# Sue1347/SMSUT-MedicalImgSegmentation

Hardware: AMD Instinct MI355X
Metric: slices/sec uganConsisTrainer step @256x256 (higher is better)
Workload: dtype f32

## Files before the change

### smsut-medicalimgsegmentation_amd/csrc/conv_mfma.hip

```cpp
#include "common.h"
#include "conv_wino.h"
#include "conv_wgrad_rr.h"
#include <stdlib.h>
#include <type_traits>

namespace {

typedef float f32x4 __attribute__((ext_vector_type(4)));

constexpr int TPB = 256;
constexpr int TW = 16;
constexpr int CK = 16;
constexpr int SPIX = 24;

#ifdef SMSUT_STAMPS
__device__ unsigned long long* g_stamps = nullptr;
__device__ int g_stamp_base = 0;
#define STAMP(i)                                                                                       \
  if (g_stamps && lane == 0 && stamp_wg >= g_stamp_base && stamp_wg < g_stamp_base + 512)                \
    g_stamps[(((stamp_wg - g_stamp_base) * 4 + wave) * 16) + (i)] = __builtin_amdgcn_s_memtime();
#else
#define STAMP(i)
#endif

// ... 151 lines not shown
        else *(float4*)(w_s + w_dst[i]) = rw[i];
      }
    }
    __syncthreads();
    if (step < 2) { STAMP(3 + 4 * step); }
    if (step + 1 < nsteps) prefetch(step + 1);
    if (step < 2) { STAMP(4 + 4 * step); }
    if constexpr (CKW == 32) {
#pragma unroll
      for (int tap = 0; tap < KK; ++tap) {
        const int kh = tap / KS, kw = tap % KS;
        h8 a[MR], b[NR];
#pragma unroll
        for (int i = 0; i < MR; ++i)
          a[i] = *(const h8*)(in_h + (((wm * MR + i) * RPT + a_row + kh) * IW + a_col + kw) * PXH + 8 * kq);
#pragma unroll
        for (int j = 0; j < NR; ++j)
          b[j] = *(const h8*)(w_h + ((size_t)tap * CO_T + (wn * NR + j) * 16 + lm) * WRH + 8 * kq);
#pragma unroll
        for (int i = 0; i < MR; ++i)
#pragma unroll
          for (int j = 0; j < NR; ++j) acc[i][j] = mfma32h(a[i], b[j], acc[i][j]);
      }
    } else if constexpr (F16 && SMSUT_F16_X32) {
      const bool hi = kq >= 2;
      const int ko = 8 * (kq & 1);
      const h8 zero8 = {(_Float16)0.f, (_Float16)0.f, (_Float16)0.f, (_Float16)0.f, (_Float16)0.f, (_Float16)0.f, (_Float16)0.f, (_Float16)0.f};
#pragma unroll
      for (int p = 0; p < (KK + 1) / 2; ++p) {
        const bool solo = 2 * p + 1 >= KK;
        const int tlo = 2 * p, thi = solo ? 2 * p : 2 * p + 1;
        const int tap = hi ? thi : tlo;
        const int kh = hi ? thi / KS : tlo / KS, kw = hi ? thi % KS : tlo % KS;
        h8 a[MR], b[NR];
#pragma unroll
        for (int i = 0; i < MR; ++i) {
          a[i] = *(const h8*)(in_h + (((wm * MR + i) * RPT + a_row + kh) * IW + a_col + kw) * SPIXH + ko);
          if (solo && hi) a[i] = zero8;
        }
#pragma unroll
        for (int j = 0; j < NR; ++j) {
          b[j] = *(const h8*)(w_h + ((size_t)tap * CO_T + (wn * NR + j) * 16 + lm) * WROWH + ko);
          if (solo && hi) b[j] = zero8;
        }
#pragma unroll
        for (int i = 0; i < MR; ++i)
#pragma unroll
          for (int j = 0; j < NR; ++j) acc[i][j] = mfma32h(a[i], b[j], acc[i][j]);
      }
    } else if constexpr (F16) {
#pragma unroll
      for (int tap = 0; tap < KK; ++tap) {
        const int kh = tap / KS, kw = tap % KS;
        h4 a[MR], b[NR];
#pragma unroll
        for (int i = 0; i < MR; ++i)
          a[i] = *(const h4*)(in_h + (((wm * MR + i) * RPT + a_row + kh) * IW + a_col + kw) * SPIXH + 4 * kq);
#pragma unroll
        for (int j = 0; j < NR; ++j)
          b[j] = *(const h4*)(w_h + ((size_t)tap * CO_T + (wn * NR + j) * 16 + lm) * WROWH + 4 * kq);
#pragma unroll
        for (int i = 0; i < MR; ++i)
#pragma unroll
          for (int j = 0; j < NR; ++j) acc[i][j] = mfma16h(a[i], b[j], acc[i][j]);
      }
    } else
#pragma unroll
    for (int tap = 0; tap < KK; ++tap) {
      const int kh = tap / KS, kw = tap % KS;
      f32x4 a[MR], b[NR];
#pragma unroll
      for (int i = 0; i < MR; ++i)
        a[i] = *(const f32x4*)(in_s + (((wm * MR + i) * RPT + a_row + kh) * IW + a_col + kw) * SPIX + 4 * kq);
#pragma unroll
      for (int j = 0; j < NR; ++j)
        b[j] = *(const f32x4*)(w_s + (((tap * 4 + kq) * CO_T) + (wn * NR + j) * 16 + lm) * 4);
#pragma unroll
      for (int s = 0; s < 4; ++s)
#pragma unroll
        for (int i = 0; i < MR; ++i)
#pragma unroll
          for (int j = 0; j < NR; ++j) acc[i][j] = mfma16(a[i][s], b[j][s], acc[i][j]);
    }
    if (step < 2) { STAMP(5 + 4 * step); }
  }
  if (F16) {
#pragma unroll
    for (int i = 0; i < MR; ++i)
#pragma unroll
      for (int j = 0; j < NR; ++j) acc[i][j] *= gi;
  }
  if (stats) {
    __syncthreads();
    float* red = smem;
#pragma unroll
    for (int j = 0; j < NR; ++j) {
      float s1 = 0.f, s2 = 0.f;
#pragma unroll
      for (int i = 0; i < MR; ++i) {
#pragma unroll
        for (int r = 0; r < 4; ++r) {
          const int p = 4 * kq + r;
          const bool ok = y0 + (wm * MR + i) * RPT + p / MW < H && x0 + p % MW < W;
          const float v = ok ? acc[i][j][r] : 0.f;
          s1 += v; s2 += v * v;
        }
      }
      s1 += __shfl_xor(s1, 16, 64); s2 += __shfl_xor(s2, 16, 64);
      s1 += __shfl_xor(s1, 32, 64); s2 += __shfl_xor(s2, 32, 64);
      if (kq == 0) {
        red[(wm * CO_T + (wn * NR + j) * 16 + lm) * 2] = s1;
        red[(wm * CO_T + (wn * NR + j) * 16 + lm) * 2 + 1] = s2;
      }
    }
    __syncthreads();
    if (tid < CO_T && co0 + tid < Ndim) {
      float s1 = 0.f, s2 = 0.f;
#pragma unroll
      for (int m = 0; m < WM; ++m) { s1 += red[(m * CO_T + tid) * 2]; s2 += red[(m * CO_T + tid) * 2 + 1]; }
      float* o = stats + (((size_t)n_img * gridDim.x + tile) * Ndim + co0 + tid) * 2;
      o[0] = s1; o[1] = s2;
    }
  }
  STAMP(10);
  const int Wo = W * osc;
#pragma unroll
  for (int i = 0; i < MR; ++i) {
#pragma unroll
    for (int j = 0; j < NR; ++j) {
      const int co = co0 + (wn * NR + j) * 16 + lm;
      if (co >= Ndim) continue;
      const bool hi = y2 && co0 + (wn * NR + j) * 16 >= split;
      const int os = !y2 ? Ndim : (hi ? Ndim - split : split);
      float* yout = (hi ? y2 : y) + (size_t)n_img * H * osc * Wo * os + (hi ? co - split : co);
#pragma unroll
      for (int r = 0; r < 4; ++r) {
        const int p = 4 * kq + r;
        const int gy_ = y0 + (wm * MR + i) * RPT + p / MW, gx_ = x0 + p % MW;
        if (gy_ < H && gx_ < W) {
          float* o = yout + ((size_t)(gy_ * osc + (tapo >> 1)) * Wo + gx_ * osc + (tapo & 1)) * os;
          *o = accum ? acc[i][j][r] + *o : acc[i][j][r];
        }
      }
    }
  }
  STAMP(11);
}

__device__ __forceinline__ float aff1(float v, float m, float r, float g, float b, float slope) {
  return lrelu_f(in_affine(v, m, r, g, b), slope);
}

constexpr int SPIXW = 20;

template <int KS, int TH, int NTN, int NCH, bool STATS, bool ACC, bool BST = false, bool DUAL = false, bool INAFF = false,
          bool F16 = false, bool K8 = false, bool SC = false, bool SC2 = false, bool N8 = false, bool WINO = false, bool O16 = false, bool I16 = false,
          bool FIN = false>
__global__ void __launch_bounds__(TPB) __attribute__((amdgpu_waves_per_eu(WINO ? 2 : 1, WINO ? 2 : 8)))
conv_mfma_fwd_p(const float* __restrict__ x, const float* __restrict__ w, float* __restrict__ y, int N, int H, int W,
                int Ndim, int tiles_x, int tiles_img, int items_per_wg, int transposed, float* __restrict__ stats,
                BstRef bst = BstRef{}, float* __restrict__ y2 = nullptr, int split = 0,
                const float* __restrict__ x2 = nullptr, AffRef aff = AffRef{}, const float* __restrict__ gsc = nullptr,
                ScRef sc = ScRef{}, FinRef fin = FinRef{}) {
  static_assert(!FIN || ((STATS || BST) && !F16 && !N8), "in-launch finalize: fp32 statistics / BST forms");
  static_assert(!SC || (STATS && !ACC && !BST && !INAFF && KS == 3), "fused shortcut: forward statistics forms");
  static_assert(!(SC && F16 && (K8 || WINO)), "fused shortcut with fp16 operands: the direct 16-channel-chunk form");
  static_assert(!SC2 || (DUAL && !STATS && !ACC && !BST && !INAFF && !K8 && !SC && KS == 3), "fused shortcut data-gradient");
  static_assert(!(SC2 && F16 && (WINO || N8)), "fused shortcut data-gradient with fp16 operands: the direct form, >= 16 result channels");
  static_assert(!N8 || (NTN == 1 && !STATS && !BST && !INAFF && !F16 && !K8 && !SC), "8 result channels: plain / accumulate / SC2 data-gradient forms");
  [[maybe_unused]] const bool nok = !N8 || (threadIdx.x & 15) < 8;
  static_assert(!K8 || (NCH == 1 && !DUAL && !INAFF && !F16 && !BST), "8-channel reduction: plain / statistics / accumulate / fused-shortcut forms");
  static_assert(!WINO || (KS == 3 && TH == 16 && !F16 && !K8 && !N8), "Winograd form: 3x3, 16-row items, fp32");
  static_assert(!O16 || ((F16 || (K8 && SC)) && !ACC && (!INAFF || I16) && (STATS != BST)),
                "fp16 storage: forward statistics forms / BST data-gradient, fp16 operands (or the 8-channel fused-shortcut form)");
  static_assert(!I16 || (F16 && STATS && !BST && !DUAL && !SC), "fp16 input: plain / input-side-IN forward statistics form, fp16 operands");
  constexpr int SPX = WINO ? SPIXW : SPIX;
  constexpr int NPOS = WINO ? 16 : KS * KS;
  static_assert(!(BST && (STATS || ACC)), "BST excludes the forward statistics and the accumulate form");
  static_assert(!INAFF || (STATS && !ACC && !BST && !DUAL), "input-side IN: forward statistics form only");
  static_assert(!DUAL || NCH % 2 == 0, "virtual cat input: two equal halves of whole 16-channel chunks");
  constexpr int KST = K8 ? 8 : (DUAL ? 8 * NCH : 16 * NCH);
  constexpr int KK = KS * KS;
  constexpr int PAD = (KS - 1) / 2;
  constexpr int IH = TH + KS - 1, IW = TW + KS - 1;
  constexpr int CO_T = 16 * NTN;
  constexpr int MR = TH / 4, NR = NTN;
  constexpr int Kdim = K8 ? 8 : 16 * NCH, K4 = Kdim / 4;
  constexpr int UQ = K8 ? 2 : 4;
  constexpr int UNITS = IH * IW * UQ;
  constexpr int NI = (UNITS + TPB - 1) / TPB;
  extern __shared__ float smem[];
  float* in_s = smem;
  float* red = smem + (IH * IW + 1) * SPX;
  float* w_s = red + 2 * 4 * CO_T * 2 + 8;
  [[maybe_unused]] float* wsc_s = w_s + NPOS * Kdim * CO_T;
  [[maybe_unused]] float* red_sc = wsc_s + Kdim * CO_T;
  [[maybe_unused]] _Float16* in_h = reinterpret_cast<_Float16*>(smem);
  [[maybe_unused]] _Float16* w_h = reinterpret_cast<_Float16*>(w_s);
  [[maybe_unused]] _Float16* wsc_h = reinterpret_cast<_Float16*>(wsc_s);
  [[maybe_unused]] const float gs = (F16 && gsc) ? gsc[0] : 1.f, gi = (F16 && gsc) ? gsc[1] : 1.f;

  const int tid = threadIdx.x;
  const int lane = tid & 63, wave = tid >> 6;
  const int lm = lane & 15, kq = lane >> 4;
  const int co0 = blockIdx.y * CO_T;
  float* const yo = (y2 && co0 >= split) ? y2 : y;
  const int os = !y2 ? Ndim : (co0 >= split ? Ndim - split : split);
  const int oc0 = (y2 && co0 >= split) ? co0 - split : co0;
  const int total_items = N * tiles_img;
  const int wg = (gridDim.x & 7) == 0 ? (int)((blockIdx.x & 7) * (gridDim.x >> 3) + (blockIdx.x >> 3)) : (int)blockIdx.x;
  const int item0 = wg * items_per_wg;
  const int item1 = min(item0 + items_per_wg, total_items);
  if (item0 >= item1) return;
  const int tiles_y = tiles_img / tiles_x;
  [[maybe_unused]] const int stamp_wg = blockIdx.y == 0 ? (int)blockIdx.x : -1;
  STAMP(0);

  if constexpr (WINO) {
    for (int u = tid; u < Kdim * CO_T; u += TPB) {
      const int n = u % CO_T, ci = u / CO_T;
      const int ng = co0 + n;
      if constexpr (SC2) {
        constexpr int Kh = Kdim / 2;
        if (ci >= Kh) {
          w_s[(((size_t)(ci >> 2)) * CO_T + n) * 4 + (ci & 3)] = sc.w[(size_t)ng * Kh + (ci - Kh)];
          continue;
        }
      }
      constexpr int KROW = SC2 ? Kdim / 2 : Kdim;
      float g[3][3];
#pragma unroll
      for (int tap = 0; tap < 9; ++tap)
        g[tap / 3][tap % 3] = !(transposed || SC2) ? w[((size_t)tap * Kdim + ci) * Ndim + ng]
                                                   : w[((size_t)(8 - tap) * Ndim + ng) * KROW + ci];
      float t[4][3];
#pragma unroll
      for (int b = 0; b < 3; ++b) {
        t[0][b] = g[0][b];
        t[1][b] = 0.5f * (g[0][b] + g[1][b] + g[2][b]);
        t[2][b] = 0.5f * (g[0][b] - g[1][b] + g[2][b]);
        t[3][b] = g[2][b];
      }
#pragma unroll
      for (int a = 0; a < 4; ++a) {
        const float uu[4] = {t[a][0], 0.5f * (t[a][0] + t[a][1] + t[a][2]), 0.5f * (t[a][0] - t[a][1] + t[a][2]), t[a][2]};
#pragma unroll
        for (int b = 0; b < 4; ++b) w_s[(((size_t)(a * 4 + b) * K4 + (ci >> 2)) * CO_T + n) * 4 + (ci & 3)] = uu[b];
      }
    }
  }
  for (int u = tid; u < (WINO ? 0 : KK * K4 * CO_T); u += TPB) {
    const int n = u % CO_T;
    const int k4 = (u / CO_T) % K4;
    const int tap = u / (CO_T * K4);
    const int ng = co0 + n;
    float4 v;
    if (N8 && n >= 8) {
      v = make_float4(0.f, 0.f, 0.f, 0.f);
    } else if constexpr (SC2) {
      constexpr int Kh = Kdim / 2;
      if (k4 < K4 / 2) v = *(const float4*)(w + ((size_t)(KK - 1 - tap) * Ndim + ng) * Kh + 4 * k4);
      else if (tap == KK / 2) v = *(const float4*)(sc.w + (size_t)ng * Kh + 4 * (k4 - K4 / 2));
      else v = make_float4(0.f, 0.f, 0.f, 0.f);
    } else if (!transposed) {
      const float* p = w + ((size_t)tap * Kdim + 4 * k4) * Ndim + ng;
      v.x = p[0]; v.y = p[Ndim]; v.z = p[2 * (size_t)Ndim]; v.w = p[3 * (size_t)Ndim];
    } else {
      v = *(const float4*)(w + ((size_t)(KK - 1 - tap) * Ndim + ng) * Kdim + 4 * k4);
    }
    if (F16) *(h4*)(w_h + ((size_t)(tap * NCH + (k4 >> 2)) * CO_T + n) * WROWH + 4 * (k4 & 3)) = to_h4(v);
    else *(float4*)(w_s + (size_t)u * 4) = v;
  }
  if constexpr (SC) {
    for (int u = tid; u < K4 * CO_T; u += TPB) {
      const int n = u % CO_T, k4 = u / CO_T;
      const float* p = sc.w + (size_t)(4 * k4) * Ndim + co0 + n;
      const float4 v = make_float4(p[0], p[Ndim], p[2 * (size_t)Ndim], p[3 * (size_t)Ndim]);
      if (F16) *(h4*)(wsc_h + ((size_t)(k4 >> 2) * CO_T + n) * WROWH + 4 * (k4 & 3)) = to_h4(v);
      else *(float4*)(wsc_s + (size_t)u * 4) = v;
    }
  }

  int u_off[NI], u_lds[NI], u_flag[NI];
  float4 rin[I16 ? 1 : NI];
  [[maybe_unused]] h4 rinh[I16 ? NI : 1];
#pragma unroll
  for (int i = 0; i < NI; ++i) {
    const int u = tid + i * TPB;
    const bool real = u < UNITS;
    const int uu = real ? u : 0;
    const int q = uu % UQ, pix = uu / UQ;
    const int iy = pix / IW, ix = pix % IW;
    u_off[i] = (iy * W + ix) * KST + 4 * q;
    u_lds[i] = real ? pix * (F16 ? SPIXH : SPX) + 4 * q : IH * IW * (F16 ? SPIXH : SPX);
    u_flag[i] = (iy < PAD ? 1 : 0) | (iy >= TH + PAD ? 2 : 0) | (ix < PAD ? 4 : 0) | (ix >= TW + PAD ? 8 : 0);
  }
  const int safe_off = (PAD * W + PAD) * KST;

  int pn = item0 / tiles_img, pty, ptx;
  { const int t = item0 - pn * tiles_img; pty = t / tiles_x; ptx = t - pty * tiles_x; }
  int cn = pn, cty = pty, ctx = ptx;
  int en = pn, ety = pty, etx = ptx;
  int pflags = 0;
  bool zero[NI];
  [[maybe_unused]] float4 a_m, a_r, a_g, a_b;

  auto prefetch = [&](int c) __attribute__((always_inline)) {
    if (c == 0) pflags = (pty == 0 ? 1 : 0) | (pty == tiles_y - 1 ? 2 : 0) | (ptx == 0 ? 4 : 0) | (ptx == tiles_x - 1 ? 8 : 0);
    const int cl = DUAL ? c % (NCH / 2 > 0 ? NCH / 2 : 1) : c;
    const int base = (((pn * H + pty * TH - PAD) * W) + ptx * TW - PAD) * KST + cl * 16;
    const float* xb = ((DUAL && c >= NCH / 2) ? x2 : x) + base;
    if constexpr (I16) {
      const _Float16* xh = reinterpret_cast<const _Float16*>(x) + base;
#pragma unroll
      for (int i = 0; i < NI; ++i) {
        zero[i] = (u_flag[i] & pflags) != 0;
        rinh[i] = *(const h4*)(xh + (zero[i] ? safe_off : u_off[i]));
      }
    } else {
#pragma unroll
      for (int i = 0; i < NI; ++i) {
        zero[i] = (u_flag[i] & pflags) != 0;
        rin[i] = *(const float4*)(xb + (zero[i] ? safe_off : u_off[i]));
      }
    }
    if (INAFF) {
      const int ch = c * 16 + 4 * (tid & 3);
      a_m = *(const float4*)(aff.mean + (size_t)pn * Kdim + ch);
// ... 50 lines not shown
      for (int j = 0; j < NR; ++j) qacc[q_][j] = (f32x4){0.f, 0.f, 0.f, 0.f};
  }
  if constexpr (SC) {
#pragma unroll
    for (int i = 0; i < MR; ++i)
#pragma unroll
      for (int j = 0; j < NR; ++j) { acs[i][j] = (f32x4){0.f, 0.f, 0.f, 0.f}; pacs[i][j] = acs[i][j]; }
  }
  [[maybe_unused]] f32x4 pold[MR][NR];
  [[maybe_unused]] float nm[NR], nr[NR], ng[NR], nb[NR];
#pragma unroll
  for (int i = 0; i < MR; ++i)
#pragma unroll
    for (int j = 0; j < NR; ++j) { acc[i][j] = (f32x4){0.f, 0.f, 0.f, 0.f}; pacc[i][j] = acc[i][j]; }

  if (BST) {
#pragma unroll
    for (int j = 0; j < NR; ++j) { ng[j] = bst.gamma[co0 + j * 16 + lm]; nb[j] = bst.beta[co0 + j * 16 + lm]; }
  }
  const int o_lane = WINO ? ((wave * MR + 2 * (kq >> 1)) * W + 8 * (kq & 1)) * os + lm : ((wave * MR) * W + 4 * kq) * os + lm;
  const int red_slot = (wave * CO_T + lm) * 2;
  auto pxo = [&](int i, int r) __attribute__((always_inline)) { return WINO ? (i >> 1) * W + 2 * r + (i & 1) : i * W + r; };

  auto epilogue = [&](int par) __attribute__((always_inline)) {
    if (F16) {
#pragma unroll
      for (int i = 0; i < MR; ++i)
#pragma unroll
        for (int j = 0; j < NR; ++j) pacc[i][j] *= gi;
    }
    if (STATS || BST) {
#pragma unroll
      for (int j = 0; j < NR; ++j) {
        float s1 = 0.f, s2 = 0.f;
#pragma unroll
        for (int i = 0; i < MR; ++i)
#pragma unroll
          for (int r = 0; r < 4; ++r) {
            if (BST) {
              const float yv = pold[i][j][r];
              const float gz = pacc[i][j][r] * lrelu_mask(in_affine(yv, nm[j], nr[j], ng[j], nb[j]), bst.slope);
              pacc[i][j][r] = gz;
              s1 += gz; s2 += gz * ((yv - nm[j]) * nr[j]);
            } else {
              const float v = pacc[i][j][r]; s1 += v; s2 += v * v;
            }
          }
        s1 += __shfl_xor(s1, 16, 64); s2 += __shfl_xor(s2, 16, 64);
        s1 += __shfl_xor(s1, 32, 64); s2 += __shfl_xor(s2, 32, 64);
        float* rd = kq == 0 ? red + par * (4 * CO_T * 2) + j * 32 + red_slot : red + 2 * 4 * CO_T * 2;
        *(float2*)rd = make_float2(s1, s2);
      }
    }
    float* yb = yo + (((size_t)en * H + ety * TH) * W + etx * TW) * os + oc0;
#pragma unroll
    for (int i = 0; i < MR; ++i)
#pragma unroll
      for (int j = 0; j < NR; ++j)
#pragma unroll
        for (int r = 0; r < 4; ++r)
          if constexpr (O16 && !BST) {
            reinterpret_cast<_Float16*>(yo)[(((size_t)en * H + ety * TH) * W + etx * TW) * os + oc0 + o_lane + pxo(i, r) * os + j * 16] =
                (_Float16)pacc[i][j][r];
          } else if (nok) yb[o_lane + pxo(i, r) * os + j * 16] = pacc[i][j][r] + (ACC ? pold[i][j][r] : 0.f);
    if constexpr (SC) {
#pragma unroll
      for (int j = 0; j < NR; ++j) {
        float s1 = 0.f, s2 = 0.f;
#pragma unroll
        for (int i = 0; i < MR; ++i)
#pragma unroll
          for (int r = 0; r < 4; ++r) { const float v = pacs[i][j][r]; s1 += v; s2 += v * v; }
        s1 += __shfl_xor(s1, 16, 64); s2 += __shfl_xor(s2, 16, 64);
        s1 += __shfl_xor(s1, 32, 64); s2 += __shfl_xor(s2, 32, 64);
        float* rd = kq == 0 ? red_sc + par * (4 * CO_T * 2) + j * 32 + red_slot : red_sc + 2 * 4 * CO_T * 2;
        *(float2*)rd = make_float2(s1, s2);
      }
      float* ys = sc.y + (((size_t)en * H + ety * TH) * W + etx * TW) * Ndim + co0;
#pragma unroll
      for (int i = 0; i < MR; ++i)
#pragma unroll
        for (int j = 0; j < NR; ++j)
#pragma unroll
          for (int r = 0; r < 4; ++r) {
            if constexpr (O16)
              reinterpret_cast<_Float16*>(sc.y)[(((size_t)en * H + ety * TH) * W + etx * TW) * Ndim + co0 + o_lane + pxo(i, r) * Ndim + j * 16] =
                  (_Float16)pacs[i][j][r];
            else ys[o_lane + pxo(i, r) * Ndim + j * 16] = pacs[i][j][r];
          }
    }
  };
  auto load_old = [&](int n_, int ty_, int tx_) __attribute__((always_inline)) {
    if (BST) {
#pragma unroll
      for (int j = 0; j < NR; ++j) {
        nm[j] = bst.mean[(size_t)n_ * Ndim + co0 + j * 16 + lm];
        nr[j] = bst.rstd[(size_t)n_ * Ndim + co0 + j * 16 + lm];
      }
    }
    if (ACC || BST) {
      const float* yb = (BST ? bst.y1 : yo) + (((size_t)n_ * H + ty_ * TH) * W + tx_ * TW) * os + oc0;
#pragma unroll
      for (int i = 0; i < MR; ++i)
#pragma unroll
        for (int j = 0; j < NR; ++j)
#pragma unroll
          for (int r = 0; r < 4; ++r) {
            if constexpr (BST && O16)
              pold[i][j][r] = (float)reinterpret_cast<const _Float16*>(bst.y1)[(((size_t)n_ * H + ty_ * TH) * W + tx_ * TW) * os + oc0 + o_lane +
                                                                              pxo(i, r) * os + j * 16];
            else pold[i][j][r] = nok ? yb[o_lane + pxo(i, r) * os + j * 16] : 0.f;
          }
    }
  };
  auto stats_out = [&](int par) __attribute__((always_inline)) {
    if ((STATS || BST) && tid < CO_T) {
      const float* rd = red + par * (4 * CO_T * 2);
      float s1 = 0.f, s2 = 0.f;
#pragma unroll
      for (int m = 0; m < 4; ++m) { s1 += rd[(m * CO_T + tid) * 2]; s2 += rd[(m * CO_T + tid) * 2 + 1]; }
      float* const po = stats + (((size_t)en * tiles_img + ety * tiles_x + etx) * Ndim + co0 + tid) * 2;
      if constexpr (FIN) st_sc1_f2(po, s1, s2);
      else *(float2*)po = make_float2(s1, s2);
      if constexpr (SC) {
        const float* rs = red_sc + par * (4 * CO_T * 2);
        float t1 = 0.f, t2 = 0.f;
#pragma unroll
        for (int m = 0; m < 4; ++m) { t1 += rs[(m * CO_T + tid) * 2]; t2 += rs[(m * CO_T + tid) * 2 + 1]; }
        float* const ps = sc.stats + (((size_t)en * tiles_img + ety * tiles_x + etx) * Ndim + co0 + tid) * 2;
        if constexpr (FIN) st_sc1_f2(ps, t1, t2);
        else *(float2*)ps = make_float2(t1, t2);
      }
    }
  };
  auto mma_chunk = [&](int c) __attribute__((always_inline)) {
    if constexpr (WINO) {
      const float* dp = in_s + (((wave * 4 + 2 * (lm >> 3)) * IW) + 2 * (lm & 7)) * SPX + 4 * kq;
      const float* wc = w_s + ((size_t)(c * 4 + kq) * CO_T + lm) * 4;
      f32x4 d1[4], d2[4], dx[4];
      if constexpr (SC2) {
        if (c >= NCH / 2) {
          const f32x4 px[4] = {*(const f32x4*)(dp + (1 * IW + 1) * SPX), *(const f32x4*)(dp + (1 * IW + 2) * SPX),
                               *(const f32x4*)(dp + (2 * IW + 1) * SPX), *(const f32x4*)(dp + (2 * IW + 2) * SPX)};
#pragma unroll
          for (int j = 0; j < NR; ++j) {
            const f32x4 bw = *(const f32x4*)(wc + (size_t)(j * 16) * 4);
#pragma unroll
            for (int q_ = 0; q_ < 4; ++q_)
#pragma unroll
              for (int s = 0; s < 4; ++s) qacc[q_][j] = mfma16(px[q_][s], bw[s], qacc[q_][j]);
          }
        }
      }
#pragma unroll
      for (int b = 0; b < 4; ++b) {
        dx[b] = *(const f32x4*)(dp + (0 * IW + b) * SPX);
        d1[b] = *(const f32x4*)(dp + (1 * IW + b) * SPX);
        d2[b] = *(const f32x4*)(dp + (2 * IW + b) * SPX);
      }
      if constexpr (SC) {
#pragma unroll
        for (int j = 0; j < NR; ++j) {
          const f32x4 bw = *(const f32x4*)(wsc_s + (((size_t)(c * 4 + kq) * CO_T) + j * 16 + lm) * 4);
#pragma unroll
          for (int s = 0; s < 4; ++s) {
            qacc[0][j] = mfma16(d1[1][s], bw[s], qacc[0][j]);
            qacc[1][j] = mfma16(d1[2][s], bw[s], qacc[1][j]);
            qacc[2][j] = mfma16(d2[1][s], bw[s], qacc[2][j]);
            qacc[3][j] = mfma16(d2[2][s], bw[s], qacc[3][j]);
          }
        }
      }
#pragma unroll
      for (int xi = 0; xi < ((SC2 && c >= NCH / 2) ? 0 : 4); ++xi) {
        if (xi == 3) {
#pragma unroll
          for (int b = 0; b < 4; ++b) dx[b] = *(const f32x4*)(dp + (3 * IW + b) * SPX);
        }
        f32x4 t[4];
#pragma unroll
        for (int b = 0; b < 4; ++b)
          t[b] = xi == 0 ? sub4(dx[b], d2[b]) : xi == 1 ? add4(d1[b], d2[b]) : xi == 2 ? sub4(d2[b], d1[b]) : sub4(d1[b], dx[b]);
        const f32x4 v[4] = {sub4(t[0], t[2]), add4(t[1], t[2]), sub4(t[2], t[1]), sub4(t[1], t[3])};
#pragma unroll
        for (int nu = 0; nu < 4; ++nu) {
          const int pos = xi * 4 + nu;
#pragma unroll
          for (int j = 0; j < NR; ++j) {
            const f32x4 b = *(const f32x4*)(wc + ((size_t)pos * K4 * CO_T + j * 16) * 4);
#pragma unroll
            for (int s = 0; s < 4; ++s)
              macc[pos][j] = mfma16(v[nu][s], b[s], macc[pos][j]);
          }
        }
      }
      if (c == NCH - 1) {
#pragma unroll
        for (int j = 0; j < NR; ++j) {
          f32x4 c0[4], c1[4];
#pragma unroll
          for (int nu = 0; nu < 4; ++nu) {
            c0[nu] = add4(add4(macc[0 + nu][j], macc[4 + nu][j]), macc[8 + nu][j]);
            c1[nu] = sub4(sub4(macc[4 + nu][j], macc[8 + nu][j]), macc[12 + nu][j]);
          }
          const f32x4 o00 = add4(add4(c0[0], c0[1]), c0[2]), o01 = sub4(sub4(c0[1], c0[2]), c0[3]);
          const f32x4 o10 = add4(add4(c1[0], c1[1]), c1[2]), o11 = sub4(sub4(c1[1], c1[2]), c1[3]);
          acc[0][j] = o00; acc[1][j] = o01; acc[2][j] = o10; acc[3][j] = o11;
#pragma unroll
          for (int p_ = 0; p_ < 16; ++p_) macc[p_][j] = (f32x4){0.f, 0.f, 0.f, 0.f};
          if constexpr (SC || SC2) {
            if constexpr (SC) { acs[0][j] = qacc[0][j]; acs[1][j] = qacc[1][j]; acs[2][j] = qacc[2][j]; acs[3][j] = qacc[3][j]; }
            else { acc[0][j] += qacc[0][j]; acc[1][j] += qacc[1][j]; acc[2][j] += qacc[2][j]; acc[3][j] += qacc[3][j]; }
#pragma unroll
            for (int q_ = 0; q_ < 4; ++q_) qacc[q_][j] = (f32x4){0.f, 0.f, 0.f, 0.f};
          }
        }
      }
      return;
    }
    if constexpr (K8) {
      const int half = kq >> 1, kk = kq & 1;
#pragma unroll
      for (int g = 0; g < (KK + 1) / 2; ++g) {
        constexpr int dummy = 0; (void)dummy;
        const int tA = 2 * g, tB = (2 * g + 1 < KK) ? 2 * g + 1 : 2 * g;
        const int t = half ? tB : tA;
        const bool live = !(half && 2 * g + 1 >= KK);
        const int toff = ((t / KS) * IW + (t % KS)) * SPIX + 4 * kk;
        f32x4 a[MR], b[NR];
#pragma unroll
        for (int i = 0; i < MR; ++i) a[i] = *(const f32x4*)(in_s + ((wave * MR + i) * IW + lm) * SPIX + toff);
#pragma unroll
        for (int j = 0; j < NR; ++j) {
          b[j] = *(const f32x4*)(w_s + (((size_t)(t * K4 + kk) * CO_T) + j * 16 + lm) * 4);
          if (!live) b[j] = (f32x4){0.f, 0.f, 0.f, 0.f};
        }
#pragma unroll
        for (int s = 0; s < 4; ++s)
#pragma unroll
          for (int i = 0; i < MR; ++i)
#pragma unroll
            for (int j = 0; j < NR; ++j) acc[i][j] = mfma16(a[i][s], b[j][s], acc[i][j]);
        if constexpr (SC) {
          if (2 * g == KK / 2) {
            f32x4 bs[NR];
#pragma unroll
            for (int j = 0; j < NR; ++j) {
              bs[j] = *(const f32x4*)(wsc_s + (((size_t)kk * CO_T) + j * 16 + lm) * 4);
              if (half) bs[j] = (f32x4){0.f, 0.f, 0.f, 0.f};
            }
#pragma unroll
            for (int s = 0; s < 4; ++s)
#pragma unroll
              for (int i = 0; i < MR; ++i)
#pragma unroll
                for (int j = 0; j < NR; ++j) acs[i][j] = mfma16(a[i][s], bs[j][s], acs[i][j]);
          }
        }
      }
      return;
    }
    if constexpr (F16 && SMSUT_F16_X32) {
      const bool sc2_half = SC2 && c >= NCH / 2;
      const bool hi = kq >= 2;
      const int ko = 8 * (kq & 1);
      const h8 zero8 = {(_Float16)0.f, (_Float16)0.f, (_Float16)0.f, (_Float16)0.f, (_Float16)0.f, (_Float16)0.f, (_Float16)0.f, (_Float16)0.f};
#pragma unroll
      for (int p = 0; p < (KK + 1) / 2; ++p) {
        if (sc2_half && p != (KK / 2) / 2) continue;
        const bool solo = 2 * p + 1 >= KK || sc2_half;
        const int tlo = sc2_half ? KK / 2 : 2 * p, thi = (2 * p + 1 < KK) ? 2 * p + 1 : 2 * p;
        const int tap = hi ? thi : tlo;
        const int kh = hi ? thi / KS : tlo / KS, kw = hi ? thi % KS : tlo % KS;
        h8 a[MR], b[NR];
#pragma unroll
        for (int i = 0; i < MR; ++i) {
          a[i] = *(const h8*)(in_h + ((wave * MR + i + kh) * IW + lm + kw) * SPIXH + ko);
          if (solo && hi) a[i] = zero8;
        }
#pragma unroll
        for (int j = 0; j < NR; ++j) {
          b[j] = *(const h8*)(w_h + ((size_t)(tap * NCH + c) * CO_T + j * 16 + lm) * WROWH + ko);
          if (solo && hi) b[j] = zero8;
        }
#pragma unroll
        for (int i = 0; i < MR; ++i)
#pragma unroll
          for (int j = 0; j < NR; ++j) acc[i][j] = mfma32h(a[i], b[j], acc[i][j]);
        if constexpr (SC) {
          if (2 * p == KK / 2 || 2 * p + 1 == KK / 2) {
            const bool mine = hi == (2 * p + 1 == KK / 2);
            h8 bs[NR];
#pragma unroll
            for (int j = 0; j < NR; ++j) {
              bs[j] = *(const h8*)(wsc_h + ((size_t)c * CO_T + j * 16 + lm) * WROWH + ko);
              if (!mine) bs[j] = zero8;
            }
#pragma unroll
            for (int i = 0; i < MR; ++i)
#pragma unroll
              for (int j = 0; j < NR; ++j) acs[i][j] = mfma32h(a[i], bs[j], acs[i][j]);
          }
        }
      }
      return;
    }
    if constexpr (F16) {
#pragma unroll
      for (int tap = 0; tap < KK; ++tap) {
        if (SC2 && c >= NCH / 2 && tap != KK / 2) continue;
        const int kh = tap / KS, kw = tap % KS;
        h4 a[MR], b[NR];
#pragma unroll
        for (int i = 0; i < MR; ++i)
          a[i] = *(const h4*)(in_h + ((wave * MR + i + kh) * IW + lm + kw) * SPIXH + 4 * kq);
#pragma unroll
        for (int j = 0; j < NR; ++j)
          b[j] = *(const h4*)(w_h + ((size_t)(tap * NCH + c) * CO_T + j * 16 + lm) * WROWH + 4 * kq);
#pragma unroll
        for (int i = 0; i < MR; ++i)
#pragma unroll
          for (int j = 0; j < NR; ++j) acc[i][j] = mfma16h(a[i], b[j], acc[i][j]);
        if constexpr (SC) {
          if (tap == KK / 2) {
            h4 bs[NR];
#pragma unroll
            for (int j = 0; j < NR; ++j) bs[j] = *(const h4*)(wsc_h + ((size_t)c * CO_T + j * 16 + lm) * WROWH + 4 * kq);
// ... 773 lines not shown
  __shared__ float4 sm[TPB];
  const int col = threadIdx.x % COLS, sl = threadIdx.x / COLS;
  const int e = (blockIdx.x * COLS + col) * 4;
  float4 t0 = make_float4(0.f, 0.f, 0.f, 0.f), t1 = t0, t2 = t0, t3 = t0;
  if (e < wsize) {
    const float* p = part + e;
    int c = sl;
    for (; c + 3 * LANES < splits; c += 4 * LANES) {
      const float4 v0 = *(const float4*)(p + (size_t)c * wsize);
      const float4 v1 = *(const float4*)(p + (size_t)(c + LANES) * wsize);
      const float4 v2 = *(const float4*)(p + (size_t)(c + 2 * LANES) * wsize);
      const float4 v3 = *(const float4*)(p + (size_t)(c + 3 * LANES) * wsize);
      t0.x += v0.x; t0.y += v0.y; t0.z += v0.z; t0.w += v0.w;
      t1.x += v1.x; t1.y += v1.y; t1.z += v1.z; t1.w += v1.w;
      t2.x += v2.x; t2.y += v2.y; t2.z += v2.z; t2.w += v2.w;
      t3.x += v3.x; t3.y += v3.y; t3.z += v3.z; t3.w += v3.w;
    }
    for (; c < splits; c += LANES) {
      const float4 v = *(const float4*)(p + (size_t)c * wsize);
      t0.x += v.x; t0.y += v.y; t0.z += v.z; t0.w += v.w;
    }
  }
  sm[threadIdx.x] = make_float4((t0.x + t1.x) + (t2.x + t3.x), (t0.y + t1.y) + (t2.y + t3.y),
                                (t0.z + t1.z) + (t2.z + t3.z), (t0.w + t1.w) + (t2.w + t3.w));
  __syncthreads();
  if (sl == 0 && e < wsize) {
    float4 t = sm[col];
    for (int l = 1; l < LANES; ++l) {
      const float4 v = sm[l * COLS + col];
      t.x += v.x; t.y += v.y; t.z += v.z; t.w += v.w;
    }
    *(float4*)(out + e) = t;
  }
}

inline void launch_sum_splits(const float* part, float* out, int wsize, int splits, hipStream_t st,
                              [[maybe_unused]] bool dbg_force = false) {
  (void)splits;
  if (wsize >= 32768) sum_splits<64><<<(wsize + 255) / 256, TPB, 0, st>>>(part, out, wsize, splits);
  else if (wsize >= 8192) sum_splits<32><<<(wsize + 127) / 128, TPB, 0, st>>>(part, out, wsize, splits);
  else sum_splits<16><<<(wsize + 63) / 64, TPB, 0, st>>>(part, out, wsize, splits);
}

template <int KS, int TH, int WM, int WN, int NTN, int MW = TW>
int launch_fwd(const ConvCall& c) {
  constexpr int IH = TH + KS - 1, IW = MW + KS - 1;
  constexpr size_t sh16 = (size_t)(IH * IW * SPIX + KS * KS * CK * 16 * NTN) * sizeof(float);
  constexpr size_t sh32 = (size_t)(IH * IW * SPIX) * sizeof(float) + (size_t)(KS * KS * 16 * NTN * 40) * sizeof(_Float16);
  constexpr size_t sh = sh16;
  static_assert(sh16 <= 64 * 1024 && (KS != 3 || MW != TW || sh32 <= 64 * 1024), "LDS budget");
  const int tiles_x = (c.W + MW - 1) / MW, tiles_y = (c.H + TH - 1) / TH;
  const bool plain_taps = c.isc == 1 && c.osc == 1 && c.G == 1 && c.ntap_out == 1;
  if (MW != TW && !plain_taps) return -1;
  const int nz = (c.Ndim + 16 * NTN - 1) / (16 * NTN);
  if (c.tiles_out) { *c.tiles_out = tiles_x * tiles_y; return 0; }
  dim3 grid(tiles_x * tiles_y, c.N, nz * c.ntap_out);
  if ((c.x2 && (!plain_taps || c.transposed_w || c.Kdim % 32 != 0)) ||
      (c.y2 && (c.osc != 1 || c.ntap_out != 1 || c.stats || c.split <= 0 || c.split >= c.Ndim || c.split % 16 != 0)))
    return -1;
  auto go = [&](auto kern, size_t lds) {
    kern<<<grid, TPB, lds, c.stream>>>((const float*)c.x, c.w, (float*)c.y, c.H, c.W, c.Kdim, c.Ndim, tiles_x, c.transposed_bits(), c.isc,
                                       c.osc, c.G, nz, c.stats, c.x2, c.y2, c.split, c.gsc);
    return 0;
  };
  if constexpr (KS == 3 && MW == TW && SMSUT_F16_X32) {
    if (c.f16_operands && c.Kdim % 32 == 0 && c.Kdim >= 32 && (!c.x2 || (c.Kdim / 2) % 32 == 0) && c.isc == 1 && c.osc == 1 && c.G == 1)
      return go(conv_mfma_fwd<KS, TH, WM, WN, NTN, true, MW, 32>, sh32);
  }
  if (c.f16_operands) return go(conv_mfma_fwd<KS, TH, WM, WN, NTN, true, MW>, sh);
  return go(conv_mfma_fwd<KS, TH, WM, WN, NTN, false, MW>, sh);
}

template <int KS, int TH, int NTN, int NCH, bool WINO = false>
constexpr size_t fwd_p_lds() {
  return (size_t)(((TH + KS - 1) * (TW + KS - 1) + 1) * (WINO ? SPIXW : SPIX) + 2 * 4 * 16 * NTN * 2 + 8 +
                  (WINO ? 16 : KS * KS) * 16 * NCH * 16 * NTN) * sizeof(float);
}


template <auto Kern>
inline int p_occupancy(size_t lds) {
  static const int occ = [lds] {
    if (lds > 64 * 1024) (void)hipFuncSetAttribute((const void*)Kern, hipFuncAttributeMaxDynamicSharedMemorySize, (int)lds);
    int o = 0;
    if (hipOccupancyMaxActiveBlocksPerMultiprocessor(&o, Kern, TPB, lds) != hipSuccess || o < 1) o = 1;
    return o;
  }();
  return occ;
}

template <int KS, int TH, int NTN, int NCH, unsigned F>
constexpr auto fwd_p_kernel =
    conv_mfma_fwd_p<KS, TH, NTN, NCH, (F & F_STATS) != 0, (F & F_ACC) != 0, (F & F_BST) != 0, (F & F_DUAL) != 0, (F & F_INAFF) != 0,
                    (F & F_F16) != 0, (F & F_K8) != 0, (F & F_SC) != 0, (F & F_SC2) != 0, (F & F_N8) != 0, (F & F_WINO) != 0,
                    (F & F_O16) != 0, (F & F_I16) != 0, (F & F_FIN) != 0>;

template <int KS, int TH, int NTN, int NCH, bool K8 = false, bool N8 = false, bool WINO = false>
int launch_fwd_p(const ConvCall& c) {
  const bool tw = c.transposed_w, acc = c.accumulate, f16 = c.f16_operands, o16 = c.out_f16, i16 = c.in_f16;
  const auto x2 = c.x2; const auto y2 = c.y2; const auto stats = c.stats;
  const auto bst = c.bst; const auto aff = c.aff; const auto sc = c.sc; const auto fin = c.fin;
  const int N = c.N, H = c.H, W = c.W, Kdim = c.Kdim, Ndim = c.Ndim, split = c.split;
  if (fin && (!fin->tickets || !fin->o0 || !fin->o1 || !stats || f16 || N8 || y2 || o16 || i16 || acc ||
              (fin->s0 && !(sc && !tw && sc->stats && fin->s1)) || (!fin->s0 && sc)))
    return -1;
  constexpr size_t sh = fwd_p_lds<KS, TH, NTN, NCH, WINO>();
  constexpr size_t sh_sc = sh + (size_t)(16 * NCH * 16 * NTN + 2 * 4 * 16 * NTN * 2 + 8) * sizeof(float);
  if constexpr (sh > (WINO ? 160 : 64) * 1024) return -1;
  else {
  if (Kdim != (K8 ? 8 : 16 * NCH) || W % TW != 0 || H % TH != 0 || (N8 ? Ndim != 8 : Ndim % (16 * NTN) != 0) ||
      (int64_t)N * H * W * (Kdim > Ndim ? Kdim : Ndim) >= (1ll << 31))
    return -1;
  if (N8 && (NTN != 1 || K8 || stats || c.tiles_out || bst || y2 || aff || f16 || !tw || (x2 && !(sc && sc->w)))) return -1;
  if (K8 && (f16 || bst || x2 || aff)) return -1;
  if (WINO && (f16 || K8 || N8)) return -1;
  const int tiles_x = W / TW, tiles_y = H / TH;
  const int tiles_img = tiles_x * tiles_y;
  if (y2 && (split <= 0 || split >= Ndim || split % (16 * NTN) != 0 || stats || bst)) return -1;
  if (x2 && !(sc && tw) && (NCH % 2 != 0 || !stats || bst || y2 || tw || acc)) return -1;
  if (aff && (!stats || bst || y2 || x2 || tw || acc)) return -1;
  const bool sc2 = sc && tw;
  if (sc2 && (K8 || KS != 3 || NCH % 2 != 0 || !x2 || stats || bst || aff || acc || (f16 && (WINO || N8)) || !sc->w)) return -1;
  if (sc && !sc2 && (KS != 3 || sh_sc > 64 * 1024 || !stats || bst || y2 || aff || tw || acc || !sc->w || !sc->y || !sc->stats ||
                     (K8 && x2) || (f16 && (K8 || WINO))))
    return -1;
  if (i16 && (!o16 || bst || x2 || sc)) return -1;
  if (o16 && !bst && (!(f16 || (K8 && sc)) || !stats || (aff && !i16) || y2 || tw || acc || (K8 && !sc) || N8 || WINO || KS != 3)) return -1;
  if (o16 && bst && (!f16 || !stats || aff || y2 || x2 || sc || acc || K8 || N8 || WINO || KS != 3)) return -1;
  if (c.tiles_out) { *c.tiles_out = tiles_img; return 0; }
  const int nz = N8 ? 1 : Ndim / (16 * NTN);
  const int64_t items = (int64_t)N * tiles_img;
  int ipw = 1;
  dim3 grid(1, nz);
  auto size_grid = [&](int occ) {
    const int64_t slots = (int64_t)device_cus() * occ;
    ipw = (int)((items * nz + slots - 1) / slots);
    if (ipw < 1) ipw = 1;
    grid.x = (unsigned)((items + ipw - 1) / ipw);
  };
  auto go = [&](auto form, size_t lds) {
    constexpr auto kern = fwd_p_kernel<KS, TH, NTN, NCH, decltype(form)::value>;
    size_grid(p_occupancy<kern>(lds));
    kern<<<grid, TPB, lds, c.stream>>>((const float*)c.x, c.w, (float*)c.y, N, H, W, Ndim, tiles_x, tiles_img, ipw, tw ? 1 : 0, stats,
                                       bst ? *bst : BstRef{}, y2, split, x2, aff ? *aff : AffRef{}, f16 ? c.gsc : nullptr,
                                       sc ? *sc : ScRef{}, fin ? *fin : FinRef{});
    return 0;
  };
  auto go_opt = [&](bool on, auto extra, auto form, size_t lds) {
    return on ? go(Form<decltype(form)::value | decltype(extra)::value>{}, lds) : go(form, lds);
  };
  auto go_plain = [&](auto form) {
    constexpr unsigned B = decltype(form)::value | (K8 ? F_K8 : 0u) | (WINO ? F_WINO : 0u);
    if constexpr (K8 && (B & (F_BST | F_DUAL | F_INAFF)) != 0) return -1;
    else {
      if constexpr ((B & (F_STATS | F_BST)) != 0 && !(B & F_ACC)) {
        if (fin) return go(Form<B | F_FIN>{}, sh);
      }
      if constexpr (!K8 && !WINO) return go_opt(f16, Form<F_F16>{}, Form<B>{}, sh);
      else return go(Form<B>{}, sh);
    }
  };
  if constexpr (N8) {
    if constexpr (NTN == 1 && !K8 && KS == 3) {
      if (sc2) {
        if constexpr (NCH % 2 == 0) return go(Form<F_DUAL | F_SC2 | F_N8>{}, sh);
        else return -1;
      }
      return go_opt(acc, Form<F_ACC>{}, Form<F_N8>{}, sh);
    } else return -1;
  } else if (sc2) {
    if constexpr (!K8 && KS == 3 && NCH % 2 == 0) {
      if (f16) {
        if constexpr (!WINO) return go(Form<F_DUAL | F_F16 | F_SC2>{}, sh);
        else return -1;
      }
      return go(Form<F_DUAL | F_SC2 | (WINO ? F_WINO : 0u)>{}, sh);
    } else return -1;
  } else if (sc) {
    if constexpr (K8 && KS == 3 && sh_sc <= 64 * 1024) {
      if (o16) return go(Form<F_STATS | F_K8 | F_SC | F_O16>{}, sh_sc);
      return go_opt(fin != nullptr, Form<F_FIN>{}, Form<F_STATS | F_K8 | F_SC>{}, sh_sc);
    } else if constexpr (!K8 && KS == 3 && sh_sc <= 64 * 1024) {
      if (f16) {
        if constexpr (!WINO) {
          if (!x2) return go_opt(o16, Form<F_O16>{}, Form<F_STATS | F_F16 | F_SC>{}, sh_sc);
          if constexpr (NCH % 2 == 0) return go_opt(o16, Form<F_O16>{}, Form<F_STATS | F_DUAL | F_F16 | F_SC>{}, sh_sc);
          else return -1;
        } else return -1;
      }
      constexpr unsigned SCW = F_STATS | F_SC | (WINO ? F_WINO : 0u);
      if (!x2) return go_opt(fin != nullptr, Form<F_FIN>{}, Form<SCW>{}, sh_sc);
      if constexpr (NCH % 2 == 0) return go_opt(fin != nullptr, Form<F_FIN>{}, Form<SCW | F_DUAL>{}, sh_sc);
      else return -1;
    } else return -1;
  } else if (aff && i16) {
    if constexpr (!K8 && !WINO && KS == 3) return go(Form<F_STATS | F_INAFF | F_F16 | F_O16 | F_I16>{}, sh);
    else return -1;
  } else if (aff) {
    return go_plain(Form<F_STATS | F_INAFF>{});
  } else if (o16 && !bst) {
    if constexpr (!K8 && !WINO && KS == 3) {
      if (!x2) return go_opt(i16, Form<F_I16>{}, Form<F_STATS | F_F16 | F_O16>{}, sh);
      if constexpr (NCH % 2 == 0) return go(Form<F_STATS | F_DUAL | F_F16 | F_O16>{}, sh);
      else return -1;
    } else return -1;
  } else if (x2) {
    if constexpr (NCH % 2 == 0) return go_plain(Form<F_STATS | F_DUAL>{});
    else return -1;
  } else if (bst && o16) {
    if constexpr (!K8 && !WINO && KS == 3) return go(Form<F_BST | F_F16 | F_O16>{}, sh);
    else return -1;
  } else if (bst) {
    if (!stats || acc) return -1;
    return go_plain(Form<F_BST>{});
  } else if (acc) {
    if (stats) return -1;
    return go_plain(Form<F_ACC>{});
  } else if (stats) return go_plain(Form<F_STATS>{});
  else return go_plain(Form<0u>{});
  }
}

inline bool fwd_p_eligible(int N, int H, int W, int Kdim, int Ndim) {
  return (Kdim == 8 || Kdim == 16 || Kdim == 32 || Kdim == 64) && W % TW == 0 && H % 8 == 0 && Ndim % 16 == 0 &&
         (int64_t)N * (H / 8) * (W / TW) * (Ndim / 16) >= 1024 && (int64_t)N * H * W * (Kdim > Ndim ? Kdim : Ndim) < (1ll << 31);
}

constexpr int WINO_L_MIN_K = 64;
inline bool wino_l_shape(int N, int H, int W, int Kdim, int Ndim) {
  return winograd_on() && Kdim >= WINO_L_MIN_K && smsut_wino_l_eligible(N, H, W, Kdim, Ndim);
}
inline bool fwd_any_eligible(int N, int H, int W, int Kdim, int Ndim, bool f16) {
  return fwd_p_eligible(N, H, W, Kdim, Ndim) || (!f16 && wino_l_shape(N, H, W, Kdim, Ndim));
}

inline int select_fwd_p(const ConvCall& c) {
  const int N = c.N, H = c.H, W = c.W, Kdim = c.Kdim, Ndim = c.Ndim;
  const bool f16 = c.f16_operands;
  const bool sc2_64 = c.sc && c.transposed_w && Kdim == 64 && fwd_p_eligible(N, H, W, Kdim, Ndim);
  if (!f16 && !sc2_64 && wino_l_shape(N, H, W, Kdim, Ndim)) return smsut_wino_l_launch(c);
  if (Ndim == 8) {
    if (Kdim == 16) return (H % 16 == 0) ? launch_fwd_p<3, 16, 1, 1, false, true>(c) : launch_fwd_p<3, 8, 1, 1, false, true>(c);
    if (Kdim == 32) return launch_fwd_p<3, 8, 1, 2, false, true>(c);
    return -1;
  }
  if (Kdim == 8) return (H % 16 == 0) ? launch_fwd_p<3, 16, 1, 1, true>(c) : launch_fwd_p<3, 8, 1, 1, true>(c);
  if (winograd_on() && !f16 && H % 16 == 0 && (Kdim == 16 || Kdim == 32))
    return Kdim == 16 ? launch_fwd_p<3, 16, 1, 1, false, false, true>(c) : launch_fwd_p<3, 16, 1, 2, false, false, true>(c);
  if (Kdim == 16 && H % 16 == 0) return launch_fwd_p<3, 16, 1, 1>(c);
  if (Kdim == 32 && Ndim % 32 == 0 && !(c.y2 && c.split % 32 != 0)) return launch_fwd_p<3, 8, 2, 2>(c);
  if (Kdim == 16) return launch_fwd_p<3, 8, 1, 1>(c);
  if (Kdim == 32) return launch_fwd_p<3, 8, 1, 2>(c);
  if (Kdim == 64) return launch_fwd_p<3, 8, 1, 4>(c);
  return -1;
}

inline bool fwd_p_n8_eligible(int N, int H, int W, int Kdim, int Ndim) {
  return Ndim == 8 && (Kdim == 16 || Kdim == 32) && W % TW == 0 && H % 8 == 0 && (int64_t)N * (H / 8) * (W / TW) >= 1024 &&
         (int64_t)N * H * W * Kdim < (1ll << 31);
}

template <int KS>
int dispatch_fwd(const ConvCall& c) {
  const int N = c.N, H = c.H, W = c.W, Kdim = c.Kdim, Ndim = c.Ndim;
  const bool plain_taps = c.isc == 1 && c.osc == 1 && c.G == 1 && c.ntap_out == 1;
  if constexpr (KS == 3) {
    if (plain_taps && fwd_any_eligible(N, H, W, Kdim, Ndim, c.f16_operands)) {
      if (select_fwd_p(c) == 0) return 0;
    }
    if (plain_taps && c.transposed_w && !c.stats && !c.tiles_out && !c.x2 && !c.y2 && !c.f16_operands &&
        fwd_p_n8_eligible(N, H, W, Kdim, Ndim)) {
      if (select_fwd_p(c) == 0) return 0;
    }
  }
  const int nt = (Ndim + 15) / 16;
  const int tx = (W + TW - 1) / TW;
  const int64_t wg16 = (int64_t)tx * ((H + 15) / 16) * N * ((nt + 1) / 2) * c.ntap_out;
  const int64_t wg8 = (int64_t)tx * ((H + 7) / 8) * N * ((nt + 1) / 2) * c.ntap_out;
  if (plain_taps && !c.f16_operands && H <= 8 && W <= 8 && H > 4) return launch_fwd<KS, 8, 4, 1, 1, 8>(c);
  if (H <= 4 && c.isc == 1 && c.osc == 1) return launch_fwd<KS, 4, 4, 1, 1>(c);
  if (nt == 1) return launch_fwd<KS, 8, 4, 1, 1>(c);
  if (wg16 >= 512) return launch_fwd<KS, 16, 4, 1, 2>(c);
  if (wg8 >= 256 && !c.transposed_w) return launch_fwd<KS, 8, 4, 1, 2>(c);
  return launch_fwd<KS, 8, 4, 1, 1>(c);
}

template <int KS>
int dispatch_fwd_cfg(int cfg, const ConvCall& c) {
  switch (cfg) {
    case 0: return launch_fwd<KS, 16, 4, 1, 1>(c);
    case 1: return launch_fwd<KS, 8, 4, 1, 1>(c);
    case 2: return launch_fwd<KS, 4, 4, 1, 1>(c);
    case 3: return launch_fwd<KS, 16, 4, 1, 2>(c);
    case 4: return launch_fwd<KS, 8, 4, 1, 2>(c);
    case 5: return launch_fwd<KS, 4, 4, 1, 2>(c);
    case 6: return launch_fwd<KS, 8, 2, 2, 4>(c);
    case 7: return launch_fwd<KS, 4, 1, 4, 4>(c);
    case 8: return launch_fwd<KS, 8, 4, 1, 4>(c);
    case 9: return launch_fwd<KS, 4, 2, 2, 4>(c);
    case 10: return launch_fwd<KS, 8, 2, 2, 2>(c);
    case 11: return launch_fwd<KS, 16, 2, 2, 2>(c);
    default: break;
  }
  if (KS == 3) {
    switch (cfg) {
      case 20: return launch_fwd_p<3, 8, 1, 1>(c);
// ... 1137 lines not shown
```

Baseline: 827.0.

## Software-pipeline Winograd inner loop with interleaved MFMA, transform, and LDS loads

For the Winograd conv form with BST or fused-shortcut variants and at most two channel chunks, the inner loop is restructured into a software pipeline. The weight loads for the next position are double-buffered, the input transforms for the next group are computed while the current MFMAs run, and sched_group_barrier hints interleave MFMA, VALU and LDS-read instructions. The aim is to hide LDS latency and transform arithmetic behind matrix instructions. This raises register pressure, and the Winograd BST form with four channel chunks is now disabled so dispatch falls back to another path.

```diff
diff --git a/smsut-medicalimgsegmentation_amd/csrc/conv_mfma.hip b/smsut-medicalimgsegmentation_amd/csrc/conv_mfma.hip
--- a/smsut-medicalimgsegmentation_amd/csrc/conv_mfma.hip
+++ b/smsut-medicalimgsegmentation_amd/csrc/conv_mfma.hip
@@ -327,6 +327,9 @@
 }
 
 constexpr int SPIXW = 20;
+#ifndef SMSUT_WINO_PIPE
+#define SMSUT_WINO_PIPE 1
+#endif
 
 template <int KS, int TH, int NTN, int NCH, bool STATS, bool ACC, bool BST = false, bool DUAL = false, bool INAFF = false,
           bool F16 = false, bool K8 = false, bool SC = false, bool SC2 = false, bool N8 = false, bool WINO = false, bool O16 = false, bool I16 = false,
@@ -349,6 +352,7 @@
   static_assert(!O16 || ((F16 || (K8 && SC)) && !ACC && (!INAFF || I16) && (STATS != BST)),
                 "fp16 storage: forward statistics forms / BST data-gradient, fp16 operands (or the 8-channel fused-shortcut form)");
   static_assert(!I16 || (F16 && STATS && !BST && !DUAL && !SC), "fp16 input: plain / input-side-IN forward statistics form, fp16 operands");
+  constexpr bool PIPE = WINO && SMSUT_WINO_PIPE != 0 && NCH <= 2 && (BST || SC);
   constexpr int SPX = WINO ? SPIXW : SPIX;
   constexpr int NPOS = WINO ? 16 : KS * KS;
   static_assert(!(BST && (STATS || ACC)), "BST excludes the forward statistics and the accumulate form");
@@ -705,13 +709,85 @@
           }
         }
       }
-#pragma unroll
-      for (int b = 0; b < 4; ++b) {
+      if constexpr (PIPE) {
+        if (!(SC2 && c >= NCH / 2)) {
+          constexpr int SG_VALU = 0x2, SG_MFMA = 0x8, SG_DSR = 0x100;
+          constexpr int VPM = NR == 1 ? 2 : 1;
+          f32x4 d3[4], uf[2][NR], vv[2][4], t[4];
+          auto ld_u = [&](int p, int sel) __attribute__((always_inline)) {
+#pragma unroll
+            for (int j = 0; j < NR; ++j) uf[sel][j] = *(const f32x4*)(wc + ((size_t)p * K4 * CO_T + j * 16) * 4);
+          };
+          auto xf_t = [&](int xi, int b) __attribute__((always_inline)) {
+            t[b] = xi == 0 ? sub4(dx[b], d2[b]) : xi == 1 ? add4(d1[b], d2[b]) : xi == 2 ? sub4(d2[b], d1[b]) : sub4(d1[b], d3[b]);
+          };
+          auto xf_v = [&](int sel, int nu) __attribute__((always_inline)) {
+            vv[sel][nu] = nu == 0 ? sub4(t[0], t[2]) : nu == 1 ? add4(t[1], t[2]) : nu == 2 ? sub4(t[2], t[1]) : sub4(t[1], t[3]);
+          };
+#pragma unroll
+          for (int b = 0; b < 4; ++b) {
+            dx[b] = *(const f32x4*)(dp + (0 * IW + b) * SPX);
+            d1[b] = *(const f32x4*)(dp + (1 * IW + b) * SPX);
+            d2[b] = *(const f32x4*)(dp + (2 * IW + b) * SPX);
+          }
+          ld_u(0, 0);
+#pragma unroll
+          for (int b = 0; b < 4; ++b) xf_t(0, b);
+#pragma unroll
+          for (int nu = 0; nu < 4; ++nu) xf_v(0, nu);
+          if constexpr (SC) {
+#pragma unroll
+            for (int j = 0; j < NR; ++j) {
+              const f32x4 bw = *(const f32x4*)(wsc_s + (((size_t)(c * 4 + kq) * CO_T) + j * 16 + lm) * 4);
+#pragma unroll
+              for (int s = 0; s < 4; ++s) {
+                qacc[0][j] = mfma16(d1[1][s], bw[s], qacc[0][j]);
+                qacc[1][j] = mfma16(d1[2][s], bw[s], qacc[1][j]);
+                qacc[2][j] = mfma16(d2[1][s], bw[s], qacc[2][j]);
+                qacc[3][j] = mfma16(d2[2][s], bw[s], qacc[3][j]);
+              }
+            }
+#pragma unroll
+            for (int m = 0; m < 16 * NR; ++m) {
+              __builtin_amdgcn_sched_group_barrier(SG_MFMA, 1, 0);
+              __builtin_amdgcn_sched_group_barrier(SG_VALU, VPM, 0);
+            }
+          }
+          __builtin_amdgcn_sched_barrier(0);
+#pragma unroll
+          for (int p = 0; p < 16; ++p) {
+            const int g = p >> 2, nu = p & 3;
+            if (p + 1 < 16) ld_u(p + 1, (p + 1) & 1);
+            if (p == 4) {
+#pragma unroll
+              for (int b = 0; b < 4; ++b) d3[b] = *(const f32x4*)(dp + (3 * IW + b) * SPX);
+            }
+            if (g < 3) {
+              if (nu < 2) { xf_t(g + 1, 2 * nu); xf_t(g + 1, 2 * nu + 1); }
+              else { xf_v((g + 1) & 1, 2 * nu - 4); xf_v((g + 1) & 1, 2 * nu - 3); }
+            }
+#pragma unroll
+            for (int j = 0; j < NR; ++j)
+#pragma unroll
+              for (int s = 0; s < 4; ++s) macc[p][j] = mfma16(vv[g & 1][nu][s], uf[p & 1][j][s], macc[p][j]);
+            if (p == 4) __builtin_amdgcn_sched_group_barrier(SG_DSR, NR + 4, 0);
+            else if (p + 1 < 16) __builtin_amdgcn_sched_group_barrier(SG_DSR, NR, 0);
+#pragma unroll
+            for (int m = 0; m < 4 * NR; ++m) {
+              __builtin_amdgcn_sched_group_barrier(SG_MFMA, 1, 0);
+              if (g < 3) __builtin_amdgcn_sched_group_barrier(SG_VALU, VPM, 0);
+            }
+            __builtin_amdgcn_sched_barrier(0);
+          }
+        }
+      }
+#pragma unroll
+      for (int b = 0; b < (PIPE ? 0 : 4); ++b) {
         dx[b] = *(const f32x4*)(dp + (0 * IW + b) * SPX);
         d1[b] = *(const f32x4*)(dp + (1 * IW + b) * SPX);
         d2[b] = *(const f32x4*)(dp + (2 * IW + b) * SPX);
       }
-      if constexpr (SC) {
+      if constexpr (SC && !PIPE) {
 #pragma unroll
         for (int j = 0; j < NR; ++j) {
           const f32x4 bw = *(const f32x4*)(wsc_s + (((size_t)(c * 4 + kq) * CO_T) + j * 16 + lm) * 4);
@@ -725,7 +801,7 @@
         }
       }
 #pragma unroll
-      for (int xi = 0; xi < ((SC2 && c >= NCH / 2) ? 0 : 4); ++xi) {
+      for (int xi = 0; xi < ((PIPE || (SC2 && c >= NCH / 2)) ? 0 : 4); ++xi) {
         if (xi == 3) {
 #pragma unroll
           for (int b = 0; b < 4; ++b) dx[b] = *(const f32x4*)(dp + (3 * IW + b) * SPX);
@@ -1805,6 +1881,7 @@
   auto go_plain = [&](auto form) {
     constexpr unsigned B = decltype(form)::value | (K8 ? F_K8 : 0u) | (WINO ? F_WINO : 0u);
     if constexpr (K8 && (B & (F_BST | F_DUAL | F_INAFF)) != 0) return -1;
+    else if constexpr (WINO && NCH == 4 && (B & F_BST) != 0) return -1;
     else {
       if constexpr ((B & (F_STATS | F_BST)) != 0 && !(B & F_ACC)) {
         if (fin) return go(Form<B | F_FIN>{}, sh);
```

After: 823.9. Within noise of the previous version (-0.4%).
